# incredible-vision/show-and-tell

Measured on AMD Instinct MI355X. Metric: images/sec (train step), higher is better.
Workload: dtype bf16

## Files before the change

show-and-tell_amd/csrc/sat_conv_ap.inc:

```
template <bool AFF>
__global__ __launch_bounds__(256, 2) void conv_ap_kernel(const ConvArgs p_) {
    const ConvArgs p = group_args(p_);
    constexpr int BM = 128, BN = 128, NT = 256, NKS = 4;
    constexpr int ABUF = BM * 128;
    constexpr int CROW = BN * 2 + 16;
    constexpr int CTILE = BM * CROW;
    constexpr int NJ = 4, RJ = 32;
    __shared__ __attribute__((aligned(16))) char smem[2 * ABUF + CTILE + (AFF ? 2048 : 0)];
    char* ctile = smem + 2 * ABUF;
    float* in_tab = (float*)(smem + 2 * ABUF + CTILE);

    const int tid = threadIdx.x;
    const int lane = tid & 63;
    const int wave = __builtin_amdgcn_readfirstlane(tid >> 6);
    const int r = lane & 31, h = lane >> 5;

    const int tile = xcd_tile();
    const int W = gridDim.x / p.tiles_n;
    const int worker = tile / p.tiles_n, tile_n = tile - worker * p.tiles_n;
    const int n0 = tile_n * BN;
    const int RT = (p.M + BM - 1) / BM;
    const int n_my = worker < RT ? (RT - worker + W - 1) / W : 0;
    if (n_my == 0) return;
    const int S = n_my * NKS;

    const int lc = tid & 7, r0 = tid >> 3;
    const int sw0 = (r0 >> 1) & 7;
    const __amdgpu_buffer_rsrc_t asrc = __builtin_amdgcn_make_buffer_rsrc(const_cast<bf16_t*>(p.A), 0, (int)(p.in_bytes), 0x00020000);
    const int a_voff = (r0 * p.Cin + ((lc ^ sw0) << 3)) * 2;
    const int a_jstep = RJ * p.Cin * 2;
    auto load_a_stage = [&](int g, u32x4 (&dst)[NJ]) {
        const int gg = g < S ? g : S - 1;
        const int m0 = (worker + (gg >> 2) * W) * BM;
        const int so = (m0 * p.Cin + (gg & 3) * 64) * 2;
#pragma unroll
        for (int j = 0; j < NJ; ++j) dst[j] = __builtin_bit_cast(u32x4, __builtin_amdgcn_raw_buffer_load_b128(asrc, a_voff, so + j * a_jstep, 0));
    };
    auto rows_ok = [&](int tile_seq) {
        const int m0 = (worker + tile_seq * W) * BM;
        unsigned ok = 0u;
#pragma unroll
        for (int j = 0; j < NJ; ++j)
            if (m0 + r0 + RJ * j < p.M) ok |= 1u << j;
        return ok;
    };

    u32x4 ar[4][NJ];
    load_a_stage(0, ar[0]);
    load_a_stage(1, ar[1]);
    load_a_stage(2, ar[2]);
    load_a_stage(3, ar[3]);
    bf16x8 wreg[NKS][4];
    {
        const __amdgpu_buffer_rsrc_t wsrc = __builtin_amdgcn_make_buffer_rsrc(
            const_cast<char*>((const char*)p.Bp + (long)((n0 >> 5) + wave) * NKS * 4096), 0, NKS * 4096, 0x00020000);
#pragma unroll
        for (int kt = 0; kt < NKS; ++kt)
#pragma unroll
            for (int ks = 0; ks < 4; ++ks)
                wreg[kt][ks] = __builtin_bit_cast(bf16x8, __builtin_amdgcn_raw_buffer_load_b128(wsrc, lane * 16, kt * 4096 + ks * 1024, 0));
    }
    f32x16 acc[4];
    const f32x16 kZero16 = {0.f, 0.f, 0.f, 0.f, 0.f, 0.f, 0.f, 0.f, 0.f, 0.f, 0.f, 0.f, 0.f, 0.f, 0.f, 0.f};

    if constexpr (AFF) {
        conv_in_table<NT>(p, in_tab);
        lds_barrier();
    }
    auto store_a_stage = [&](int kt, int buf, u32x4 (&src)[NJ], unsigned ok) {
        char* at0 = smem + buf * ABUF + r0 * 128 + (lc << 4);
        if constexpr (AFF) {
            const float* ts = in_tab + kt * 64 + ((lc ^ sw0) << 3);
            const InTab tab = in_tab_fetch(ts, p.Cin);
#pragma unroll
            for (int j = 0; j < NJ; ++j) {
                u32x4 w = src[j];
                w = bn_relu_chunk(w, tab, (ok >> j) & 1u);
                *(u32x4*)(at0 + j * (RJ * 128)) = w;
            }
        } else {
#pragma unroll
            for (int j = 0; j < NJ; ++j) *(u32x4*)(at0 + j * (RJ * 128)) = src[j];
        }
    };

    int a_off[4];
#pragma unroll
    for (int ks = 0; ks < 4; ++ks) a_off[ks] = frag_off(r, h, ks);

    const __amdgpu_buffer_rsrc_t csrc = __builtin_amdgcn_make_buffer_rsrc(p.C, 0, (int)((long)p.M * p.ldc * 2), 0x00020000);
    const int c_voff = ((tid >> 4) * (int)p.ldc + n0 + (tid & 15) * 8) * 2;
    const int c_istep = 16 * (int)p.ldc * 2;
    const int colw = wave * 32 + r;
    float s_run = 0.0f, q_run = 0.0f;
    unsigned ok_cur = rows_ok(0);
    store_a_stage(0, 0, ar[0], ok_cur);
    load_a_stage(4, ar[0]);

    for (int ts_ = 0; ts_ < n_my; ++ts_) {
        const unsigned ok_next = rows_ok(ts_ + 1);
        const int tile_m = worker + ts_ * W;
        const int m0 = tile_m * BM;
        auto step = [&](auto kt_tag) {
            constexpr int KT = decltype(kt_tag)::value, K1 = (KT + 1) & 3;
            const int g = ts_ * NKS + KT;
            lds_barrier();
            if (g + 1 < S) store_a_stage(K1, K1 & 1, ar[K1], KT == 3 ? ok_next : ok_cur);
            load_a_stage(g + 5, ar[K1]);
            const char* st = smem + (KT & 1) * ABUF;
#pragma unroll
            for (int ks = 0; ks < 4; ++ks) {
                bf16x8 fa[4];
#pragma unroll
                for (int i = 0; i < 4; ++i) fa[i] = *(const bf16x8*)(st + a_off[ks] + i * 4096);
#pragma unroll
                for (int i = 0; i < 4; ++i)
                    acc[i] = __builtin_amdgcn_mfma_f32_32x32x16_bf16(fa[i], wreg[KT][ks], (KT == 0 && ks == 0) ? kZero16 : acc[i], 0, 0, 0);
            }
        };
        step(std::integral_constant<int, 0>{});
        step(std::integral_constant<int, 1>{});
        step(std::integral_constant<int, 2>{});
        step(std::integral_constant<int, 3>{});

        if (p.stat_partial || p.acc) {
            float s = 0.0f, q = 0.0f;
#pragma unroll
            for (int i = 0; i < 4; ++i)
#pragma unroll
                for (int e = 0; e < 16; ++e) {
                    const float v = acc[i][e];
                    s += v;
                    q += v * v;
                }
            if (p.stat_partial) {
                const float s2 = s + __shfl_xor(s, 32, 64), q2 = q + __shfl_xor(q, 32, 64);
                if (h == 0) {
                    stat_slab_store(p.stat_partial, tile_m, p.N, s2, q2, n0, colw);
                }
            }
            s_run += s;
            q_run += q;
        }
#pragma unroll
        for (int i = 0; i < 4; ++i)
#pragma unroll
            for (int e = 0; e < 16; ++e) {
                const int row = acc_row(i, e, h);
                *(bf16_t*)(ctile + row * CROW + colw * 2) = (bf16_t)acc[i][e];
            }
        lds_barrier();
#pragma unroll
        for (int it = 0; it < 8; ++it) {
            const int qid = tid + it * NT;
            const int row = qid >> 4, cc = qid & 15;
            const u32x4 v = *(const u32x4*)(ctile + row * CROW + cc * 16);
            __builtin_amdgcn_raw_buffer_store_b128(__builtin_bit_cast(__attribute__((__vector_size__(4 * sizeof(unsigned)))) unsigned, v), csrc,
                                                   c_voff, m0 * (int)p.ldc * 2 + it * c_istep, 17);
        }
        ok_cur = ok_next;
    }
    if (p.acc) {
        const float s2 = s_run + __shfl_xor(s_run, 32, 64), q2 = q_run + __shfl_xor(q_run, 32, 64);
        if (h == 0) {
            stat_acc_add(p.acc, p.N, s2, q2, n0, colw);
        }
    }
}

bool ap_ok(const ConvArgs& a) {
    return a.Bp != nullptr && a.linear && a.K == 256 && a.Cin == 256 && (a.N % 128) == 0 && !a.residual && !a.out_scale &&
           a.in_bytes > 0 && a.in_bytes < 0x7ffffff0L && a.ldc == a.N && (long)a.M * a.ldc * 2 < 0x7ffffff0L;
}

int ap_workers(const ConvArgs& a) {
    const int tiles_n = a.N / 128, rt = sat_cdiv(a.M, 128);
    int wmax = 256 / tiles_n;
    if (wmax < 1) wmax = 1;
    const int tpw = sat_cdiv(rt, wmax);
    return sat_cdiv(rt, tpw);
}

int launch_ap(ConvArgs& a, int groups, hipStream_t s) {
    if (!ap_ok(a)) return SAT_ERR_UNSUPPORTED;
    a.tiles_n = a.N / 128;
    return launch_conv(a.in_affine ? conv_ap_kernel<true> : conv_ap_kernel<false>, dim3(ap_workers(a) * a.tiles_n, groups), dim3(256), 0, s, a);
}
```

show-and-tell_amd/csrc/sat_conv_aw.inc:

```
template <bool AFF, int NW, bool RES>
__global__ __launch_bounds__(NW * 64, 2) void conv_aw_kernel(const ConvArgs p_) {
    const ConvArgs p = group_args(p_);
    constexpr int BM = 128, BN = NW * 32, NT = NW * 64, PD = 3;
    constexpr int ABUF = BM * 128;
    constexpr int CROW = BN * 2 + 16;
    constexpr int NJ = BM * 8 / NT;
    constexpr int RJ = NT / 8;
    constexpr int TAB = (3 * ABUF > BM * CROW) ? 3 * ABUF : BM * CROW;
    __shared__ __attribute__((aligned(16))) char smem[TAB + (AFF ? 4096 : 0)];

    const int tid = threadIdx.x;
    const int lane = tid & 63;
    const int wave = __builtin_amdgcn_readfirstlane(tid >> 6);
    const int r = lane & 31, h = lane >> 5;

    const int tile = xcd_tile();
    const int tile_m = tile / p.tiles_n, tile_n = tile - tile_m * p.tiles_n;
    const int m0 = tile_m * BM, n0 = tile_n * BN;
    const int nk = p.Cin >> 6;

    const int lc = tid & 7, r0 = tid >> 3;
    const int sw0 = (r0 >> 1) & 7;
    const __amdgpu_buffer_rsrc_t asrc = __builtin_amdgcn_make_buffer_rsrc(const_cast<bf16_t*>(p.A), 0, (int)(p.in_bytes), 0x00020000);
    int a_voff[NJ];
    unsigned a_ok = 0u;
#pragma unroll
    for (int j = 0; j < NJ; ++j) {
        const int grow = m0 + r0 + RJ * j;
        long pix;
        if (p.linear) {
            pix = (long)grow * p.sW;
        } else {
            const int hw = p.Hout * p.Wout;
            const int n = grow / hw;
            const int rem = grow - n * hw;
            const int ho = rem / p.Wout;
            const int wo = rem - ho * p.Wout;
            pix = (long)n * p.sN + (long)(ho * p.stride) * p.sH + (long)(wo * p.stride) * p.sW;
        }
        const bool ok = grow < p.M;
        a_voff[j] = ok ? (int)((pix + ((lc ^ sw0) << 3)) * 2) : 0x7ffffff0;
        if (ok) a_ok |= 1u << j;
    }
    auto load_a_stage = [&](int g, u32x4 (&dst)[NJ]) {
        const int gs = (g < nk ? g : nk - 1) * 128;
#pragma unroll
        for (int j = 0; j < NJ; ++j) dst[j] = __builtin_bit_cast(u32x4, __builtin_amdgcn_raw_buffer_load_b128(asrc, a_voff[j], gs, 0));
    };

    const __amdgpu_buffer_rsrc_t wsrc = __builtin_amdgcn_make_buffer_rsrc(
        const_cast<char*>((const char*)p.Bp + (long)((n0 >> 5) + wave) * nk * 4096), 0, nk * 4096, 0x00020000);
    const int wlane = lane * 16;
    auto load_b = [&](int g, int ks) {
        return __builtin_bit_cast(bf16x8, __builtin_amdgcn_raw_buffer_load_b128(wsrc, wlane, (g < nk ? g : nk - 1) * 4096 + ks * 1024, 0));
    };

    u32x4 ar[3][NJ];
    load_a_stage(0, ar[0]);
    load_a_stage(1, ar[1]);
    load_a_stage(2, ar[2]);
    bf16x8 bq[PD][4];
#pragma unroll
    for (int s = 0; s < PD; ++s)
#pragma unroll
        for (int ks = 0; ks < 4; ++ks) bq[s][ks] = load_b(s, ks);

    f32x16 acc[4];
#pragma unroll
    for (int i = 0; i < 4; ++i)
#pragma unroll
        for (int e = 0; e < 16; ++e) acc[i][e] = 0.0f;

    float* in_tab = (float*)(smem + TAB);
    if constexpr (AFF) {
        conv_in_table<NT>(p, in_tab);
        lds_barrier();
    }
    auto store_a_stage = [&](int g, int buf, u32x4 (&src)[NJ]) {
        char* at0 = smem + buf * ABUF + r0 * 128 + (lc << 4);
        if constexpr (AFF) {
            const float* ts = in_tab + g * 64 + ((lc ^ sw0) << 3);
            const bool live = g < nk;
            const float* tq = live ? ts : in_tab;
            const InTab tab = in_tab_fetch(tq, p.Cin);
#pragma unroll
            for (int j = 0; j < NJ; ++j) {
                u32x4 w = src[j];
                w = bn_relu_chunk(w, tab, (a_ok >> j) & 1u);
                *(u32x4*)(at0 + j * (RJ * 128)) = w;
            }
        } else {
#pragma unroll
            for (int j = 0; j < NJ; ++j) *(u32x4*)(at0 + j * (RJ * 128)) = src[j];
        }
    };

    int a_off[4];
#pragma unroll
    for (int ks = 0; ks < 4; ++ks) a_off[ks] = frag_off(r, h, ks);

    store_a_stage(0, 0, ar[0]);
    load_a_stage(3, ar[0]);

    auto step = [&](int g, auto u_tag, auto tail_tag) {
        constexpr int U = decltype(u_tag)::value, U1 = (U + 1) % 3;
        constexpr bool TAIL = decltype(tail_tag)::value;
        lds_barrier();
        store_a_stage(g + 1, U1, ar[U1]);
        if constexpr (!TAIL) load_a_stage(g + 4, ar[U1]);
        const char* st = smem + U * ABUF;
#pragma unroll
        for (int ks = 0; ks < 4; ++ks) {
            bf16x8 fa[4];
#pragma unroll
            for (int i = 0; i < 4; ++i) fa[i] = *(const bf16x8*)(st + a_off[ks] + i * 4096);
            const bf16x8 b = bq[U][ks];
#pragma unroll
            for (int i = 0; i < 4; ++i) acc[i] = __builtin_amdgcn_mfma_f32_32x32x16_bf16(fa[i], b, acc[i], 0, 0, 0);
            if constexpr (!TAIL) bq[U][ks] = load_b(g + PD, ks);
        }
    };
    constexpr int ITS = BM * (BN / 8) / NT;
    u32x4 resv[RES ? ITS : 1];
    auto fetch_residual = [&]() {
        if constexpr (RES) {
            const __amdgpu_buffer_rsrc_t rsrc = __builtin_amdgcn_make_buffer_rsrc(const_cast<bf16_t*>(p.residual), 0, (int)((long)p.M * p.ldc * 2), 0x00020000);
#pragma unroll
            for (int it = 0; it < ITS; ++it) {
                const int qid = tid + it * NT;
                const int row = qid / (BN / 8), cc = qid % (BN / 8);
                resv[it] = __builtin_bit_cast(u32x4, __builtin_amdgcn_raw_buffer_load_b128(rsrc, (int)(((long)(m0 + row) * p.ldc + n0 + cc * 8) * 2), 0, 0));
            }
        }
    };
    const int rem = nk % 3 == 0 ? 3 : nk % 3;
    int g = 0;
    for (; g + 3 <= nk - rem; g += 3) {
        step(g, std::integral_constant<int, 0>{}, std::false_type{});
        step(g + 1, std::integral_constant<int, 1>{}, std::false_type{});
        step(g + 2, std::integral_constant<int, 2>{}, std::false_type{});
    }
    const int colw = wave * 32 + r;
    float osc = 1.0f, osh = 0.0f;
    if (p.out_scale && n0 + colw < p.N) { osc = p.out_scale[n0 + colw]; osh = p.out_shift[n0 + colw]; }
    fetch_residual();
    step(g, std::integral_constant<int, 0>{}, std::true_type{});
    if (rem > 1) step(g + 1, std::integral_constant<int, 1>{}, std::true_type{});
    if (rem > 2) step(g + 2, std::integral_constant<int, 2>{}, std::true_type{});
    lds_barrier();

    if (p.stat_partial || p.acc) {
        float s = 0.0f, q = 0.0f;
#pragma unroll
        for (int i = 0; i < 4; ++i)
#pragma unroll
            for (int e = 0; e < 16; ++e) {
                const float v = acc[i][e];
                s += v;
                q += v * v;
            }
        lane_halves(s, q);
        const int col = n0 + colw;
        if (h == 0 && col < p.N) {
            if (p.acc) {
                stat_acc_add(p.acc, p.N, s, q, col);
            }
            if (p.stat_partial) {
                stat_slab_store(p.stat_partial, tile_m, p.N, s, q, col);
            }
        }
    }
    {
        const bool relu_now = p.out_relu && !RES;
#pragma unroll
        for (int i = 0; i < 4; ++i)
#pragma unroll
            for (int e = 0; e < 16; ++e) {
                const int row = acc_row(i, e, h);
                float v = acc[i][e];
                if (p.out_scale) v = v * osc + osh;
                if (relu_now) v = fmaxf(v, 0.0f);
                *(bf16_t*)(smem + row * CROW + colw * 2) = (bf16_t)v;
            }
    }
    lds_barrier();
#pragma unroll
    for (int it = 0; it < ITS; ++it) {
        const int qid = tid + it * NT;
        const int row = qid / (BN / 8), cc = qid % (BN / 8);
        const int grow = m0 + row, gcol = n0 + cc * 8;
        if (grow < p.M && gcol < p.N) {
            if constexpr (RES) {
                const bf16x8 c = *(const bf16x8*)(smem + row * CROW + cc * 16);
                const bf16x8 z = __builtin_bit_cast(bf16x8, resv[it]);
                bf16x8 o;
#pragma unroll
                for (int k = 0; k < 8; ++k) {
                    float v = (float)c[k] + (float)z[k];
                    if (p.out_relu) v = fmaxf(v, 0.0f);
                    o[k] = (bf16_t)v;
                }
                store16_wt(p.C + (long)grow * p.ldc + gcol, __builtin_bit_cast(u32x4, o));
            } else {
                store16_wt(p.C + (long)grow * p.ldc + gcol, *(const u32x4*)(smem + row * CROW + cc * 16));
            }
        }
    }
}

bool aw_ok(const ConvArgs& a, int nw) {
    return a.Bp != nullptr && a.KH == 1 && a.KW == 1 && a.pad == 0 && a.padw == 0 && (a.Cin % 64) == 0 && a.K == a.Cin && (a.N % (nw * 32)) == 0 &&
           (!a.in_affine || (a.Cin <= 512 && a.linear)) && a.in_bytes > 0 && a.in_bytes < 0x7ffffff0L;
}

template <int NW>
int launch_aw(ConvArgs& a, int groups, hipStream_t s) {
    if (!aw_ok(a, NW)) return SAT_ERR_UNSUPPORTED;
    a.tiles_n = a.N / (NW * 32);
    static constexpr ConvKernel kKernel[2][2] = {{conv_aw_kernel<false, NW, false>, conv_aw_kernel<true, NW, false>},
                                                 {conv_aw_kernel<false, NW, true>, conv_aw_kernel<true, NW, true>}};
    const bool res = a.residual != nullptr;
    const bool fits = !res || (long)a.M * a.ldc * 2 < 0x7ffffff0L;
    return launch_conv(fits ? kKernel[res][a.in_affine] : nullptr, dim3(sat_cdiv(a.M, 128) * a.tiles_n, groups), dim3(NW * 64), 0, s, a);
}
```

show-and-tell_amd/csrc/sat_conv_tile.h:

```cpp
#pragma once
#include "sat_bn_stats.h"

typedef float f32x2 __attribute__((ext_vector_type(2)));
typedef __bf16 bf16x2 __attribute__((ext_vector_type(2)));
typedef short s16x2 __attribute__((ext_vector_type(2)));

template <int N> __device__ __forceinline__ void wait_vmcnt() { asm volatile("s_waitcnt vmcnt(%0)" ::"n"(N) : "memory"); }
__device__ __forceinline__ void raw_barrier() {
    __builtin_amdgcn_s_barrier();
    asm volatile("" ::: "memory");
}
__device__ __forceinline__ void lds_barrier() {
    asm volatile("s_waitcnt lgkmcnt(0)" ::: "memory");
    raw_barrier();
}

__device__ __forceinline__ int swz_of(int row) { return (row >> 1) & 7; }
__device__ __forceinline__ int swz_chunk(int c, int row) { return c ^ swz_of(row); }
__device__ __forceinline__ int frag_off(int r, int h, int ks) { return r * 128 + (swz_chunk(2 * ks + h, r) << 4); }

struct InTab { f32x4 s0, s1, t0, t1; };
__device__ __forceinline__ InTab in_tab_fetch(const float* ts, int cin) {
    return {*(const f32x4*)ts, *(const f32x4*)(ts + 4), *(const f32x4*)(ts + cin), *(const f32x4*)(ts + cin + 4)};
}
__device__ __forceinline__ u32x4 bn_relu_chunk(u32x4 w, const InTab& t, bool keep = true) {
#pragma unroll
    for (int q = 0; q < 4; ++q) {
        f32x2 sc2, sh2, f;
        sc2[0] = q < 2 ? t.s0[2 * q] : t.s1[2 * q - 4]; sc2[1] = q < 2 ? t.s0[2 * q + 1] : t.s1[2 * q - 3];
        sh2[0] = q < 2 ? t.t0[2 * q] : t.t1[2 * q - 4]; sh2[1] = q < 2 ? t.t0[2 * q + 1] : t.t1[2 * q - 3];
        f[0] = __uint_as_float(w[q] << 16);
        f[1] = __uint_as_float(w[q] & 0xffff0000u);
        f = __builtin_elementwise_fma(f, sc2, sh2);
        const s16x2 pk = __builtin_bit_cast(s16x2, __builtin_convertvector(f, bf16x2));
        const s16x2 zero2 = {0, 0};
        w[q] = keep ? __builtin_bit_cast(unsigned int, __builtin_elementwise_max(pk, zero2)) : 0u;
    }
    return w;
}

__device__ __forceinline__ void lane_halves(float& s, float& q) {
    s += __shfl_xor(s, 32, 64);
    q += __shfl_xor(q, 32, 64);
}

__device__ __forceinline__ int acc_row(int i, int e, int h) { return i * 32 + (e & 3) + 8 * (e >> 2) + 4 * h; }
```

show-and-tell_amd/tune.py:

```python
import json
import os

from . import _lib as L

TABLE_PATH = os.path.join(os.path.dirname(os.path.abspath(__file__)), "tune", "gfx950.json")

_committed = None


def mode():
    v = os.environ.get("SAT_AUTOTUNE", "").strip().lower()
    if v in ("0", "off"):
        return "off"
    if v in ("1", "time"):
        return "time"
    if v == "force":
        return "force"
    return "table"


def committed():
    global _committed
    if _committed is None:
        tab = {}
        try:
            with open(os.environ.get("SAT_TUNE_TABLE") or TABLE_PATH) as f:
                doc = json.load(f)
            lib = L.load()
            if int(doc.get("abi", -1)) == L.ABI_VERSION and int(doc.get("variants", -1)) == int(lib.sat_conv_num_variants()):
                tab = {str(k): int(v) for k, v in doc.get("table", {}).items()}
        except (OSError, ValueError):
            tab = {}
        _committed = tab
    return _committed


def _fused_bits(o):
    return (1 if (o.stat_partial or o.stat_acc) else 0) + (2 if (o.scale0 or o.stat_acc1) else 0) + \
           (4 if o.scale1 else 0) + (8 if o.in1 else 0) + (16 if o.w_packed else 0)


def layer_key(o):
    return "%d,%d,%d,%d,%d,%d,%d,%d,%d,%d" % (o.Hin, o.Win, o.Cin, o.Hout, o.Wout, o.Cout, o.KH, o.KW, o.stride, _fused_bits(o))


def geom_key(o):
    return "%d,%d,%d,%d,%d,%d,%d,%d,%d,%d,%d" % (o.N, o.Hin, o.Win, o.Cin, o.Hout, o.Wout, o.Cout, o.KH, o.KW, o.stride,
                                                 _fused_bits(o))


def tune_key(o, want_sig=None):
    return "%s,g%d%s" % (geom_key(o), max(int(o.groups), 1), "" if want_sig is None else ",s%d" % want_sig)


def matches(variant, want):
    lib = L.load()
    return (lib.sat_conv_variant_family(variant) if want >= 100000 else lib.sat_conv_variant_signature(variant)) == want


def load_tables():
    m = mode()
    table = dict(committed()) if m in ("table", "time") else {}
    tune_file = os.environ.get("SAT_TUNE_FILE")
    if m in ("time", "force") and tune_file and os.path.exists(tune_file):
        try:
            with open(tune_file) as f:
                table.update({str(k): int(v) for k, v in json.load(f).items()})
        except ValueError:
            pass
    return table


def assign(ops, n_ops, want_of=None):
    table = load_tables() if mode() != "off" else {}
    missing = []
    for i in range(n_ops):
        o = ops[i]
        if o.kind != L.OP_CONV or o.dtype != L.SAT_BF16:
            continue
        want = want_of(o) if want_of else None
        v = table.get(tune_key(o, want))
        if v is None or v < 1 or (want is not None and not matches(int(v), want)):
            missing.append(i)
            o.variant = -want if want is not None else 0
        else:
            o.variant = int(v)
    return missing


def defaults(ops, idx, want_of=None):
    lib = L.load()
    for i in idx:
        o = ops[i]
        want = want_of(o) if want_of else None
        o.variant = 0
        o.variant = int(lib.sat_conv_default_variant(o, -1 if want is None else int(want)))


def save(ops, n_ops, want_of=None):
    tune_file = os.environ.get("SAT_TUNE_FILE")
    if not tune_file or mode() not in ("time", "force"):
        return
    table = {}
    if os.path.exists(tune_file):
        try:
            with open(tune_file) as f:
                table.update(json.load(f))
        except ValueError:
            pass
    for i in range(n_ops):
        o = ops[i]
        if o.kind == L.OP_CONV and o.dtype == L.SAT_BF16 and int(o.variant) > 0:
            table[tune_key(o, want_of(o) if want_of else None)] = int(o.variant)
    tmp = "%s.%d.tmp" % (tune_file, os.getpid())
    with open(tmp, "w") as f:
        json.dump(table, f, indent=0, sort_keys=True)
    os.replace(tmp, tune_file)
```

Measured before the change: 19020.

## Software-pipeline LDS fragment reads against MFMA in AP and AW conv kernels

Replaces compiler-scheduled LDS fragment loads with inline-asm ds_read_b128 and explicit lgkmcnt waits, so the next k-slice's A fragments are prefetched while the current MFMAs run. In the AW kernel the A staging goes one stage deeper (two stores ahead) with double-buffered fragment registers and a barrier that leaves reads in flight. In the AP kernel without affine preprocessing, the first fragments are read before the barrier-free first step. It also adds a stderr warning when the tuning table is ignored. This raises register pressure and leans on hand-placed waitcnt accounting, which could be subtly wrong or hurt occupancy.

```diff
diff --git a/show-and-tell_amd/csrc/sat_conv_ap.inc b/show-and-tell_amd/csrc/sat_conv_ap.inc
--- a/show-and-tell_amd/csrc/sat_conv_ap.inc
+++ b/show-and-tell_amd/csrc/sat_conv_ap.inc
@@ -5,6 +5,7 @@
     constexpr int ABUF = BM * 128;
     constexpr int CROW = BN * 2 + 16;
     constexpr int CTILE = BM * CROW;
+    constexpr bool EARLY = !AFF;
     constexpr int NJ = 4, RJ = 32;
     __shared__ __attribute__((aligned(16))) char smem[2 * ABUF + CTILE + (AFF ? 2048 : 0)];
     char* ctile = smem + 2 * ABUF;
@@ -93,30 +94,48 @@
     const int c_istep = 16 * (int)p.ldc * 2;
     const int colw = wave * 32 + r;
     float s_run = 0.0f, q_run = 0.0f;
+    unsigned a_rd[4];
+#pragma unroll
+    for (int ks = 0; ks < 4; ++ks) a_rd[ks] = lds_addr(smem) + a_off[ks];
+    bf16x8 fa[4];
     unsigned ok_cur = rows_ok(0);
     store_a_stage(0, 0, ar[0], ok_cur);
     load_a_stage(4, ar[0]);
+    lds_barrier();
+    if constexpr (EARLY) frag_read4<0>(fa, a_rd[0]);
 
     for (int ts_ = 0; ts_ < n_my; ++ts_) {
         const unsigned ok_next = rows_ok(ts_ + 1);
         const int tile_m = worker + ts_ * W;
         const int m0 = tile_m * BM;
         auto step = [&](auto kt_tag) {
-            constexpr int KT = decltype(kt_tag)::value, K1 = (KT + 1) & 3;
+            constexpr int KT = decltype(kt_tag)::value, K1 = (KT + 1) & 3, BUF = (KT & 1) * ABUF;
             const int g = ts_ * NKS + KT;
-            lds_barrier();
+            if constexpr (KT != 0) {
+                lds_barrier();
+                if constexpr (EARLY) frag_read4<BUF>(fa, a_rd[0]);
+            }
             if (g + 1 < S) store_a_stage(K1, K1 & 1, ar[K1], KT == 3 ? ok_next : ok_cur);
             load_a_stage(g + 5, ar[K1]);
-            const char* st = smem + (KT & 1) * ABUF;
-#pragma unroll
-            for (int ks = 0; ks < 4; ++ks) {
-                bf16x8 fa[4];
-#pragma unroll
-                for (int i = 0; i < 4; ++i) fa[i] = *(const bf16x8*)(st + a_off[ks] + i * 4096);
-#pragma unroll
-                for (int i = 0; i < 4; ++i)
+            if constexpr (!EARLY) frag_read4<BUF>(fa, a_rd[0]);
+#pragma unroll
+            for (int ks = 0; ks < 4; ++ks)
+#pragma unroll
+                for (int i = 0; i < 4; ++i) {
+                    if (ks < 3) frag_wait1<3>(fa[i]);
+                    else if (i == 0) frag_wait1<3>(fa[i]);
+                    else if (i == 1) frag_wait1<2>(fa[i]);
+                    else if (i == 2) frag_wait1<1>(fa[i]);
+                    else frag_wait1<0>(fa[i]);
                     acc[i] = __builtin_amdgcn_mfma_f32_32x32x16_bf16(fa[i], wreg[KT][ks], (KT == 0 && ks == 0) ? kZero16 : acc[i], 0, 0, 0);
-            }
+                    if (ks < 3) {
+                        if (i == 0) frag_read1<BUF>(fa[i], a_rd[ks < 3 ? ks + 1 : 0]);
+                        else if (i == 1) frag_read1<BUF + 4096>(fa[i], a_rd[ks < 3 ? ks + 1 : 0]);
+                        else if (i == 2) frag_read1<BUF + 8192>(fa[i], a_rd[ks < 3 ? ks + 1 : 0]);
+                        else frag_read1<BUF + 12288>(fa[i], a_rd[ks < 3 ? ks + 1 : 0]);
+                    }
+                }
+            __builtin_amdgcn_sched_barrier(0);
         };
         step(std::integral_constant<int, 0>{});
         step(std::integral_constant<int, 1>{});
@@ -150,6 +169,7 @@
                 *(bf16_t*)(ctile + row * CROW + colw * 2) = (bf16_t)acc[i][e];
             }
         lds_barrier();
+        if constexpr (EARLY) frag_read4<0>(fa, a_rd[0]);
 #pragma unroll
         for (int it = 0; it < 8; ++it) {
             const int qid = tid + it * NT;
@@ -160,6 +180,7 @@
         }
         ok_cur = ok_next;
     }
+    if constexpr (EARLY) frag_wait<0>(fa);
     if (p.acc) {
         const float s2 = s_run + __shfl_xor(s_run, 32, 64), q2 = q_run + __shfl_xor(q_run, 32, 64);
         if (h == 0) {
diff --git a/show-and-tell_amd/csrc/sat_conv_aw.inc b/show-and-tell_amd/csrc/sat_conv_aw.inc
--- a/show-and-tell_amd/csrc/sat_conv_aw.inc
+++ b/show-and-tell_amd/csrc/sat_conv_aw.inc
@@ -99,26 +99,45 @@
 #pragma unroll
     for (int ks = 0; ks < 4; ++ks) a_off[ks] = frag_off(r, h, ks);
 
+    unsigned a_rd[4];
+#pragma unroll
+    for (int ks = 0; ks < 4; ++ks) a_rd[ks] = lds_addr(smem) + a_off[ks];
+    bf16x8 fa0[4], fa1[4];
+
     store_a_stage(0, 0, ar[0]);
     load_a_stage(3, ar[0]);
+    store_a_stage(1, 1, ar[1]);
+    load_a_stage(4, ar[1]);
+    lds_barrier();
+    frag_read4<0>(fa0, a_rd[0]);
 
     auto step = [&](int g, auto u_tag, auto tail_tag) {
-        constexpr int U = decltype(u_tag)::value, U1 = (U + 1) % 3;
+        constexpr int U = decltype(u_tag)::value, U1 = (U + 1) % 3, U2 = (U + 2) % 3;
         constexpr bool TAIL = decltype(tail_tag)::value;
-        lds_barrier();
-        store_a_stage(g + 1, U1, ar[U1]);
-        if constexpr (!TAIL) load_a_stage(g + 4, ar[U1]);
-        const char* st = smem + U * ABUF;
-#pragma unroll
-        for (int ks = 0; ks < 4; ++ks) {
-            bf16x8 fa[4];
-#pragma unroll
-            for (int i = 0; i < 4; ++i) fa[i] = *(const bf16x8*)(st + a_off[ks] + i * 4096);
-            const bf16x8 b = bq[U][ks];
-#pragma unroll
-            for (int i = 0; i < 4; ++i) acc[i] = __builtin_amdgcn_mfma_f32_32x32x16_bf16(fa[i], b, acc[i], 0, 0, 0);
-            if constexpr (!TAIL) bq[U][ks] = load_b(g + PD, ks);
-        }
+        if constexpr (!TAIL) {
+            store_a_stage(g + 2, U2, ar[U2]);
+            load_a_stage(g + 5, ar[U2]);
+        } else if constexpr (U == 0) {
+            if (g + 2 < nk) store_a_stage(g + 2, U2, ar[U2]);
+        }
+        auto substep = [&](auto ks_tag, bf16x8 (&cur)[4]) {
+            constexpr int KS = decltype(ks_tag)::value;
+            frag_wait<4>(cur);
+            const bf16x8 b = bq[U][KS];
+#pragma unroll
+            for (int i = 0; i < 4; ++i) acc[i] = __builtin_amdgcn_mfma_f32_32x32x16_bf16(cur[i], b, acc[i], 0, 0, 0);
+            if constexpr (!TAIL) bq[U][KS] = load_b(g + PD, KS);
+        };
+        frag_read4<U * ABUF>(fa1, a_rd[1]);
+        substep(std::integral_constant<int, 0>{}, fa0);
+        frag_read4<U * ABUF>(fa0, a_rd[2]);
+        substep(std::integral_constant<int, 1>{}, fa1);
+        frag_read4<U * ABUF>(fa1, a_rd[3]);
+        substep(std::integral_constant<int, 2>{}, fa0);
+        frag_read4<U1 * ABUF>(fa0, a_rd[0]);
+        substep(std::integral_constant<int, 3>{}, fa1);
+        __builtin_amdgcn_sched_barrier(0);
+        lds_barrier_keep<4>();
     };
     constexpr int ITS = BM * (BN / 8) / NT;
     u32x4 resv[RES ? ITS : 1];
@@ -147,6 +166,7 @@
     step(g, std::integral_constant<int, 0>{}, std::true_type{});
     if (rem > 1) step(g + 1, std::integral_constant<int, 1>{}, std::true_type{});
     if (rem > 2) step(g + 2, std::integral_constant<int, 2>{}, std::true_type{});
+    frag_wait<0>(fa0);
     lds_barrier();
 
     if (p.stat_partial || p.acc) {
diff --git a/show-and-tell_amd/csrc/sat_conv_tile.h b/show-and-tell_amd/csrc/sat_conv_tile.h
--- a/show-and-tell_amd/csrc/sat_conv_tile.h
+++ b/show-and-tell_amd/csrc/sat_conv_tile.h
@@ -18,6 +18,38 @@
 __device__ __forceinline__ int swz_of(int row) { return (row >> 1) & 7; }
 __device__ __forceinline__ int swz_chunk(int c, int row) { return c ^ swz_of(row); }
 __device__ __forceinline__ int frag_off(int r, int h, int ks) { return r * 128 + (swz_chunk(2 * ks + h, r) << 4); }
+
+typedef __attribute__((address_space(3))) char* lds_cptr_t;
+__device__ __forceinline__ unsigned lds_addr(const char* p) { return (unsigned)(unsigned long)(lds_cptr_t)p; }
+template <int IMM>
+__device__ __forceinline__ void frag_read4(bf16x8 (&f)[4], unsigned addr) {
+    static_assert(IMM >= 0 && IMM + 3 * 4096 < 65536, "ds_read offset field");
+    asm volatile("ds_read_b128 %0, %4 offset:%5\n\t"
+                 "ds_read_b128 %1, %4 offset:%6\n\t"
+                 "ds_read_b128 %2, %4 offset:%7\n\t"
+                 "ds_read_b128 %3, %4 offset:%8"
+                 : "=&v"(f[0]), "=&v"(f[1]), "=&v"(f[2]), "=&v"(f[3])
+                 : "v"(addr), "n"(IMM), "n"(IMM + 4096), "n"(IMM + 8192), "n"(IMM + 12288)
+                 : "memory");
+}
+template <int N>
+__device__ __forceinline__ void frag_wait(bf16x8 (&f)[4]) {
+    asm volatile("s_waitcnt lgkmcnt(%4)" : "+v"(f[0]), "+v"(f[1]), "+v"(f[2]), "+v"(f[3]) : "n"(N) : "memory");
+}
+template <int IMM>
+__device__ __forceinline__ void frag_read1(bf16x8& f, unsigned addr) {
+    static_assert(IMM >= 0 && IMM < 65536, "ds_read offset field");
+    asm volatile("ds_read_b128 %0, %1 offset:%2" : "=&v"(f) : "v"(addr), "n"(IMM) : "memory");
+}
+template <int N>
+__device__ __forceinline__ void frag_wait1(bf16x8& f) {
+    asm volatile("s_waitcnt lgkmcnt(%1)" : "+v"(f) : "n"(N) : "memory");
+}
+template <int N>
+__device__ __forceinline__ void lds_barrier_keep() {
+    asm volatile("s_waitcnt lgkmcnt(%0)" ::"n"(N) : "memory");
+    raw_barrier();
+}
 
 struct InTab { f32x4 s0, s1, t0, t1; };
 __device__ __forceinline__ InTab in_tab_fetch(const float* ts, int cin) {
diff --git a/show-and-tell_amd/tune.py b/show-and-tell_amd/tune.py
--- a/show-and-tell_amd/tune.py
+++ b/show-and-tell_amd/tune.py
@@ -1,5 +1,6 @@
 import json
 import os
+import sys
 
 from . import _lib as L
 
@@ -23,14 +24,24 @@
     global _committed
     if _committed is None:
         tab = {}
+        path = os.environ.get("SAT_TUNE_TABLE") or TABLE_PATH
+        why = None
         try:
-            with open(os.environ.get("SAT_TUNE_TABLE") or TABLE_PATH) as f:
+            with open(path) as f:
                 doc = json.load(f)
             lib = L.load()
-            if int(doc.get("abi", -1)) == L.ABI_VERSION and int(doc.get("variants", -1)) == int(lib.sat_conv_num_variants()):
+            abi, nvar = int(doc.get("abi", -1)), int(doc.get("variants", -1))
+            if abi == L.ABI_VERSION and nvar == int(lib.sat_conv_num_variants()):
                 tab = {str(k): int(v) for k, v in doc.get("table", {}).items()}
-        except (OSError, ValueError):
+            else:
+                why = "it is stamped abi %d / %d variants, the library is abi %d / %d variants" % (
+                    abi, nvar, L.ABI_VERSION, int(lib.sat_conv_num_variants()))
+        except (OSError, ValueError) as e:
             tab = {}
+            why = "%s: %s" % (type(e).__name__, e)
+        if why is not None:
+            print("show-and-tell_amd.tune: conv tuning table %s ignored (%s): every conv runs its default variant" % (path, why),
+                  file=sys.stderr)
         _committed = tab
     return _committed
 
```

New measurement: 19010. About the same (-0.1%).
